# aghasemzadeh/OpenMPL

Hardware: AMD Instinct MI355X
Metric: poses/sec (V=4, J=17, batch=1024 per GPU) fp32 (higher is better)
Workload: dtype f32; 1 GPU; Human3.6M config: V=4 J=17 batch=1024 fp32, CHOSEN flag set, depth 12, DIM 32, heads 8; global_batch=1024, parallelism=single GPU

## Files before the change

### openmpl_amd/csrc/common.hpp

```cpp
#pragma once
#include <stdio.h>
#include <hip/hip_runtime.h>
#include <stdint.h>
#include <stdlib.h>

#include <atomic>
#include <mutex>

#include "../../include/mpl_hip.h"

namespace mpl {

inline const char* lab_getenv(const char* name) {
#ifdef MPL_LAB
    return getenv(name);
#else
    (void)name;
    return nullptr;
#endif
}

typedef _Float16 mpl_f16x8 __attribute__((ext_vector_type(8)));
typedef _Float16 mpl_f16x2 __attribute__((ext_vector_type(2)));
__device__ __forceinline__ void split2_f16(const float (&x)[8], mpl_f16x8& hi, mpl_f16x8& lo) {
    typedef unsigned u4 __attribute__((ext_vector_type(4)));
    u4 h, l;
#pragma unroll
    for (int p = 0; p < 4; ++p) {
        const mpl_f16x2 hp = {(_Float16)x[2 * p], (_Float16)x[2 * p + 1]};
        h[p] = __builtin_bit_cast(unsigned, hp);
        unsigned d;
        asm("v_fma_mixlo_f16 %0, %1, -1.0, %2 op_sel_hi:[1,0,0]\n\t"
            "v_fma_mixhi_f16 %0, %1, -1.0, %3 op_sel:[1,0,0] op_sel_hi:[1,0,0]"
            : "=&v"(d) : "v"(h[p]), "v"(x[2 * p]), "v"(x[2 * p + 1]));
        l[p] = d;
    }
    hi = __builtin_bit_cast(mpl_f16x8, h);
    lo = __builtin_bit_cast(mpl_f16x8, l);
}


typedef float f32x4 __attribute__((ext_vector_type(4)));

constexpr int kWave = 64;

__device__ __forceinline__ f32x4 mfma16(float a, float b, f32x4 c) {
    return __builtin_amdgcn_mfma_f32_16x16x4f32(a, b, c, 0, 0, 0);
}

__device__ __forceinline__ f32x4 mfma16_k16(const float4& a, const float4& b, f32x4 c) {
    c = mfma16(a.x, b.x, c);
    c = mfma16(a.y, b.y, c);
    c = mfma16(a.z, b.z, c);
    c = mfma16(a.w, b.w, c);
    return c;
}

__device__ __forceinline__ float xor16_add(float v) {
    float a = v, b = v;
    asm volatile("s_nop 1\n\tv_permlane16_swap_b32 %0, %1\n\ts_nop 1" : "+v"(a), "+v"(b));
    return a + b;
}
__device__ __forceinline__ float xor32_add(float v) {
    float a = v, b = v;
    asm volatile("s_nop 1\n\tv_permlane32_swap_b32 %0, %1\n\ts_nop 1" : "+v"(a), "+v"(b));
    return a + b;
}

__device__ __forceinline__ float wave_sum(float v) {
#pragma unroll
    for (int o = 32; o > 0; o >>= 1) v += __shfl_xor(v, o, 64);
    return v;
}

__device__ __forceinline__ void dma16(const float* g, unsigned lds_dst) {
    unsigned keep;
    asm volatile(
        "s_mov_b32 %0, m0\n\t"
        "s_mov_b32 m0, %2\n\t"
        "s_nop 0\n\t"
        "global_load_lds_dwordx4 %1, off\n\t"
        "s_mov_b32 m0, %0"
        : "=&s"(keep)
        : "v"(g), "s"(lds_dst)
        : "memory");
}

__device__ __forceinline__ float gelu_erf(float x) { return 0.5f * x * (1.0f + erff(x * 0.70710678118654752440f)); }
__device__ __forceinline__ float gelu_as_scaled(float x, float hs);
__device__ __forceinline__ float gelu_as(float x) { return gelu_as_scaled(x, 0.5f); }
__device__ __forceinline__ float gelu_as_scaled(float x, float hs) {
    const float z = x * 0.70710678118654752440f, az = fabsf(z);
    const float t = __builtin_amdgcn_rcpf(fmaf(0.3275911f, az, 1.0f));
    float pl = fmaf(1.061405429f, t, -1.453152027f);
    pl = fmaf(pl, t, 1.421413741f);
    pl = fmaf(pl, t, -0.284496736f);
    pl = fmaf(pl, t, 0.254829592f);
    const float e = __builtin_amdgcn_exp2f(-1.4426950408889634f * az * az);
    const float h = hs * x, ah = fabsf(h);
    return fmaf(-ah, (pl * t) * e, h + ah);
}


__device__ __forceinline__ float4 ld4(const float* p) { return *reinterpret_cast<const float4*>(p); }
__device__ __forceinline__ void st4(float* p, const float4& v) { *reinterpret_cast<float4*>(p) = v; }

constexpr double FINITE_MAX = 1.79769313486231570e308;
__device__ __forceinline__ bool takes_part(double w) { return w > 0.0 && w <= FINITE_MAX; }

struct ProfScope {
    ProfScope(int kind, hipStream_t s);
    ~ProfScope();
    int slot;
    hipStream_t stream;
};

int device_cu_count(int* cus);

inline int hip_check_launch() {
    hipError_t e = hipGetLastError();
    if (e != hipSuccess) fprintf(stderr, "mpl_hip: kernel launch failed: %s\n", hipGetErrorString(e));
    return e == hipSuccess ? MPL_OK : MPL_E_LAUNCH;
}

template <auto KERNEL>
int kernel_lds_once(int lds, int threads = 0) {
    static std::atomic<bool> done[64];
    int dev = 0;
    if (hipGetDevice(&dev) != hipSuccess || dev < 0 || dev >= 64) return MPL_E_LAUNCH;
    if (done[dev].load(std::memory_order_acquire)) return MPL_OK;
    const void* k = reinterpret_cast<const void*>(KERNEL);
    if (hipFuncSetAttribute(k, hipFuncAttributeMaxDynamicSharedMemorySize, lds) != hipSuccess) return MPL_E_LAUNCH;
    int per_cu = 0;
    if (threads > 0 && (hipOccupancyMaxActiveBlocksPerMultiprocessor(&per_cu, k, threads, lds) != hipSuccess || per_cu < 1))
        return MPL_E_UNSUPPORTED;
    done[dev].store(true, std::memory_order_release);
    return MPL_OK;
}

inline int ln_stat_slices(int K) { return (K % 136 == 0) ? K / 136 : 1; }
int launch_row_stats(const float* x, int M, int K, int ldx, float* stats, hipStream_t s);
int launch_ln_gemm(const float* A, int lda, const float* stats, const float* ln_w, const float* ln_b, float eps,
                   const float* W, const float* bias, const float* R, int ldr, float* C, int ldc, int M, int N, int K,
                   int epi, float* stats_out, hipStream_t s);
bool qkv_attention_fusable(int n_tok, int dim, int heads);
bool ln_gemm_rows_ok(long long M, int K, int lda);
int launch_ln_qkv_attention(const float* x, int M, int D, const float* stats, const float* ln_w, const float* ln_b,
                            float eps, const float* W, const float* bias, int n_tok, int heads, float* att,
                            hipStream_t s);
unsigned* device_error_word(int dev);
int device_error_pending(int dev);
void device_error_clear(int dev);
void set_fault_injection(int phase);
int take_fault_injection();
int refuse_stream_capture(hipStream_t s);
void h2_set_spin_log2(int log2_polls);
int stack_mode();
constexpr int H2_CTR_PER_TILE = 4;
constexpr int H2_XCC_WORDS = 256;
inline int h2_err_index(int n_tiles) { return H2_CTR_PER_TILE * n_tiles + H2_XCC_WORDS; }
int h2_stack_form_code(int M, int D, int n_tok, int np, int cus);
hipEvent_t stack_chain_event(int dev);
std::mutex& stack_chain_mutex(int dev);
bool h2_shape_ok(int N, int K);
size_t h2_operand_bytes(int N, int K, int np = 2);
const float* h2_out_scale(const unsigned short* op, int N, int K);
size_t h2_act_bytes(int M, int K, int rpt, int np = 2);
int h2_rows_per_tile(int n_tok);
bool h2_attention_fusable(int n_tok, int dim, int heads);
void h2_set_debug_buffer(unsigned long long* p);
int launch_pack_h2(const float* W, int N, int K, const float* ln_w, const float* ln_b, const float* bias, const float* in_scale,
                   unsigned short* dst, hipStream_t s);
int launch_h2_entry(const float* X, int M, int K, int ldx, float* stats, unsigned* counters, int n_counters,
                    const unsigned short* const* ops, int n_apps, hipStream_t s);
int launch_h2_pack_rows(const float* X, int M, int K, int ldx, int rpt, unsigned short* dst, float* sc, hipStream_t s);
int launch_h2_gemm(const float* X, const unsigned short* A2, const float* a_inv, const unsigned short* W2, bool ln, const float* stats,
                   float eps, const float* R, int ldr, float* C, int ldc, unsigned short* C2, float* stats_out,
                   int M, int N, int K, int rpt, int epi, hipStream_t s);
int launch_h2_qkv_attention(const float* X, const unsigned short* W2, const float* stats, float eps, int M, int D, int n_tok,
                            int heads, unsigned short* att2, hipStream_t s);
int launch_h2_stack(float* x, int M, int D, int n_tok, int heads, const unsigned short* const* ops, int n_apps,
                    unsigned short* att2, unsigned short* hid2, float* stats, unsigned* counters, float eps, int stop_after,
                    hipStream_t s);
int launch_pack_b1(const float* W, int N, int K, const float* ln_w, const float* ln_b, const float* bias, unsigned short* dst,
                   hipStream_t s);
int launch_b1_entry(const float* X, int M, int K, int ldx, int rpt, unsigned short* x16, float* stats, unsigned* counters,
                    int n_counters, hipStream_t s);
int launch_b1_gemm(const unsigned short* A1, const unsigned short* W1, bool ln, const float* stats, float eps, const float* R, int ldr,
                   float* C, int ldc, unsigned short* C1, float* stats_out, int M, int N, int K, int rpt, int epi, hipStream_t s);
int launch_b1_qkv_attention(const unsigned short* x16, const unsigned short* W1, const float* stats, float eps, int M, int D, int n_tok,
                            int heads, unsigned short* att1, hipStream_t s);
int launch_b1_stack(float* x, unsigned short* x16, int M, int D, int n_tok, int heads, const unsigned short* const* ops, int n_apps,
                    unsigned short* att1, unsigned short* hid1, float* stats, unsigned* counters, float eps, int stop_after,
                    hipStream_t s);
int b1a_ld(int K);
size_t b1a_operand_bytes(int N, int K);
int launch_pack_b1a(const float* W, int N, int K, const float* ln_w, const float* ln_b, const float* bias, unsigned short* dst,
                    hipStream_t s);
int launch_b1a_rows(const float* X, int M, int K, unsigned short* dst, hipStream_t s);
int launch_b1a_gemm(const float* X, int ldx, const unsigned short* A16, int lda, const unsigned short* W16, const float* stats, float eps,
                    const float* R, void* C, int ldc, int M, int N, int K, int epi, hipStream_t s);
bool sm_stack_ok(int M, int D, int n_tok, int H, int n_apps, int n_blocks, int cus);
size_t sm_stack_ws_bytes(int M, int D);
int sm_stack_max_rows();
int launch_sm_stack(float* x, int n_seq, int n_tok, int D, int H, const mpl_block_weights* blocks, const uint8_t* schedule, int n_apps,
                    void* ws, size_t ws_bytes, const unsigned** err_ws, int spin_log2, hipStream_t s);
int launch_token_attention(const float* qkv, int n_seq, int n_tok, int dim, int heads, float* out, hipStream_t s);
bool token_attention_ok(int n_tok, int hd);
bool token_attention_wide_ok(int n_tok, int hd);
int launch_token_attention_wide(const float* qkv, int n_seq, int n_tok, int dim, int heads, float* out, hipStream_t s);
int launch_token_attention_bf16(const float* qkv, int n_seq, int n_tok, int dim, int heads, unsigned short* out16, int ldo, hipStream_t s);
int launch_spt(const mpl_config* cfg, const mpl_weights* w, const mpl_inputs* in, float* xs, int use_packed, hipStream_t s);
int launch_spt_any(const mpl_config* cfg, const mpl_weights* w, const mpl_inputs* in, float* xs, hipStream_t s);
int spt_form(const mpl_config* cfg, int batch, int use_packed, int cus, int* spw);
size_t spt_any_row_bytes(int d);
int spt_any_seq_cap(int J, int d);
size_t spt_pack_bytes();
int launch_spt_pack(const mpl_block_weights* bw_host, unsigned short* dst, int fold_q, hipStream_t s);
int launch_d32_qkv(const float* x, int M, const unsigned short* pack, float* qkv, hipStream_t s);
int launch_d32_mlp(float* x, const float* att, int M, const unsigned short* pack, hipStream_t s);
int launch_fuse_head(const mpl_config* cfg, const mpl_weights* w, const float* x, int batch, float* out, float* y_out,
                     const unsigned* err_ws, hipStream_t s);
int launch_layernorm_rows(const float* x, int M, int K, int ldx, const float* g, const float* b, float eps, float* y,
                          int ldy, hipStream_t s);
int launch_view_norm(const mpl_config* cfg, const mpl_weights* w, const float* x, int batch, float* xn, hipStream_t s);
int launch_linear_act(const float* xa, int Ka, int lda, const float* xb, int Kb, int ldb, int M, const float* W, int ldw,
                      const float* bias, int N, const float* bn_w, const float* bn_b, const float* bn_mean,
                      const float* bn_var, float bn_eps, int relu, float* y, int ldy, hipStream_t s);

int launch_pose_metrics(const float* out, const float* tgt, const float* wgt, int B, int J, const float* scale3,
                        const float* offset3, unsigned skip_mask, float* res, hipStream_t s);

size_t eval_state_bytes(int n_sel, int n_groups);
int launch_eval_reset(void* state, int n_sel, int n_groups, hipStream_t s);
// ... 94 lines not shown
```

### openmpl_amd/csrc/spt_packed.hip

```cpp
#include "spt_pack.hpp"
#include "spt_stage.hpp"

namespace mpl {

constexpr int ATS = 36;
constexpr int HS = 68;
constexpr int KV_F = SJ * SH * SEQ * 4;
constexpr int SPT3_RING_BYTES = (ROWS * XS + 2 * KV_F + ROWS * ATS) * 4;
constexpr int SPT3_LDS_BYTES = 160 * 1024;
constexpr int SPT3_HID_OFF = 3072;
constexpr int SPT3_Q_OFF = 20480;
static_assert(SPT3_HID_OFF + ROWS * HS <= 2 * KV_F + ROWS * ATS, "HID does not fit its alias");
static_assert((SPT3_HID_OFF + ROWS * HS - 2 * KV_F) * 4 <= SPT3_Q_OFF, "HID reaches into the staged qkv weights");
static_assert(SPT3_Q_OFF + 12 * 1024 <= ROWS * ATS * 4, "staged qkv weights do not fit behind HID in ATT");
static_assert(SPT3_RING_BYTES + 8 * 1024 + 2 * SPT3_NPAR * 4 <= SPT3_LDS_BYTES, "spare LDS too small");

typedef float f32x2 __attribute__((ext_vector_type(2)));

__device__ inline float spt_window_scale(float v) {
    if (!(v > 0.f) || !(v < 3.0e38f)) return 1.0f;
    int e;
    (void)frexpf(32768.0f / v, &e);
    e = e - 1 < -100 ? -100 : (e - 1 > 100 ? 100 : e - 1);
    return ldexpf(1.0f, e);
// ... 82 lines not shown
        for (int j = 0; j < 8; ++j) x[j] = src[j] * sw[n];
        sf16x8 hi, lo;
        spt_split2(x, hi, lo);
        frag[(size_t)(u * 2) * 64 + lane] = hi;
        frag[(size_t)(u * 2 + 1) * 64 + lane] = lo;
    }
}

int launch_spt_pack(const mpl_block_weights* bw_host, unsigned short* dst, int fold_q, hipStream_t s) {
    const mpl_block_weights* b = bw_host;
    if (!b || !dst || !b->qkv_w || !b->proj_w || !b->fc1_w || !b->fc2_w || !b->qkv_b || !b->proj_b || !b->fc1_b || !b->fc2_b ||
        !b->ln1_w || !b->ln1_b || !b->ln2_w || !b->ln2_b)
        return MPL_E_INVALID;
    ProfScope prof(MPL_K_PACK, s);
    hipLaunchKernelGGL(spt_pack_kernel, dim3(1), dim3(256), 0, s, b->qkv_w, b->qkv_b, b->ln1_w, b->ln1_b, b->proj_w, b->proj_b, b->fc1_w,
                       b->fc1_b, b->ln2_w, b->ln2_b, b->fc2_w, b->fc2_b, reinterpret_cast<char*>(dst), fold_q);
    return hip_check_launch();
}

size_t spt_pack_bytes() { return SPT_PACK_BYTES; }

template <int N>
struct SptInt { static constexpr int value = N; };

template <int KS, bool LN, bool GELU, int NCT, int AST, int DST, int LO, int HI>
__device__ __forceinline__ void spt_linear_role(const float* A, float* D, const char* wsec, const float* par, int col0, float hs,
                                                int lane) {
    if constexpr (HI > LO) {
        constexpr int M0 = LO / NCT, NM = (HI - 1) / NCT - M0 + 1;
        const int li = lane & 15, kq = lane >> 4;
        sf16x8 w[NCT][KS][2];
        float4 bc[NCT], sc[NCT];
#pragma unroll
        for (int n = 0; n < NCT; ++n) {
            if (HI - LO < NCT && (n - LO % NCT + NCT) % NCT >= HI - LO) continue;
#pragma unroll
            for (int ks = 0; ks < KS; ++ks) spt_load_unit(wsec, n * KS + ks, lane, w[n][ks]);
            bc[n] = ::mpl::ld4(par + col0 + 16 * n + 4 * kq);
            sc[n] = ::mpl::ld4(par + SPT_NCOL + col0 + 16 * n + 4 * kq);
        }
        const float* a0 = A + li * AST + 8 * kq;
        float* d0 = D + li * DST + 4 * kq;
        float4 raw[KS][2], res[NCT];
        auto read_tile = [&](int i) {
            const int m = M0 + i;
#pragma unroll
            for (int ks = 0; ks < KS; ++ks) {
                raw[ks][0] = ::mpl::ld4(a0 + m * 16 * AST + 32 * ks);
                raw[ks][1] = ::mpl::ld4(a0 + m * 16 * AST + 32 * ks + 4);
            }
            if (!GELU) {
#pragma unroll
                for (int n = 0; n < NCT; ++n)
                    if (NCT * m + n >= LO && NCT * m + n < HI) res[n] = ::mpl::ld4(d0 + m * 16 * DST + 16 * n);
            }
        };
        read_tile(0);
#pragma unroll
        for (int i = 0; i < NM; ++i) {
            const int m = M0 + i;
            sf16x8 ah[KS], al[KS];
#pragma unroll
            for (int ks = 0; ks < KS; ++ks) {
                if (LN) {
                    spt_ln_split(raw[ks][0], raw[ks][1], ah[ks], al[ks]);
                } else {
                    const float4 x0 = raw[ks][0], x1 = raw[ks][1];
                    const float y[8] = {x0.x, x0.y, x0.z, x0.w, x1.x, x1.y, x1.z, x1.w};
                    spt_split2(y, ah[ks], al[ks]);
                }
            }
            float4 x[NCT];
#pragma unroll
            for (int n = 0; n < NCT; ++n) x[n] = res[n];
            if (i + 1 < NM) read_tile(i + 1);
            f32x4 c[NCT];
#pragma unroll
            for (int n = 0; n < NCT; ++n) c[n] = f32x4{0.f, 0.f, 0.f, 0.f};
#pragma unroll
            for (int n = 0; n < NCT; ++n) {
                if (NCT * m + n < LO || NCT * m + n >= HI) continue;
#pragma unroll
                for (int ks = 0; ks < KS; ++ks) c[n] = mfma3(w[n][ks], ah[ks], al[ks], c[n]);
            }
#pragma unroll
            for (int n = 0; n < NCT; ++n) {
                if (NCT * m + n < LO || NCT * m + n >= HI) continue;
                float* dd = d0 + m * 16 * DST + 16 * n;
                if (GELU)
                    st4(dd, float4{gelu_as_scaled(fmaf(c[n][0], sc[n].x, bc[n].x), hs), gelu_as_scaled(fmaf(c[n][1], sc[n].y, bc[n].y), hs),
                                   gelu_as_scaled(fmaf(c[n][2], sc[n].z, bc[n].z), hs), gelu_as_scaled(fmaf(c[n][3], sc[n].w, bc[n].w), hs)});
                else
                    st4(dd, float4{x[n].x + fmaf(c[n][0], sc[n].x, bc[n].x), x[n].y + fmaf(c[n][1], sc[n].y, bc[n].y),
                                   x[n].z + fmaf(c[n][2], sc[n].z, bc[n].z), x[n].w + fmaf(c[n][3], sc[n].w, bc[n].w)});
            }
        }
    }
}
#define SPT_ROLE(W, MTS, KS, LN, GELU, NCT, AST, DST, ...) \
    spt_linear_role<KS, LN, GELU, NCT, AST, DST, ((MTS) * (NCT) * (W)) / NWAVE, ((MTS) * (NCT) * ((W) + 1)) / NWAVE>(__VA_ARGS__)
#define SPT_BY_WAVE(wv, ...)                          \
    switch (wv) {                                     \
        case 0: SPT_ROLE(0, __VA_ARGS__); break;      \
        case 1: SPT_ROLE(1, __VA_ARGS__); break;      \
        case 2: SPT_ROLE(2, __VA_ARGS__); break;      \
        case 3: SPT_ROLE(3, __VA_ARGS__); break;      \
        case 4: SPT_ROLE(4, __VA_ARGS__); break;      \
        case 5: SPT_ROLE(5, __VA_ARGS__); break;      \
        case 6: SPT_ROLE(6, __VA_ARGS__); break;      \
        default: SPT_ROLE(7, __VA_ARGS__); break;     \
    }


template <int SS>
__global__ __launch_bounds__(NTHR, 1) void spt3_kernel(const SptParams p) {
    constexpr int RLIVE = SJ * SS;
    constexpr int MTS = (RLIVE + 15) / 16;
    constexpr int NT = (MTS + 3) / 4;
    extern __shared__ __attribute__((aligned(16))) float smem[];
    float* X = smem;
    float* Kb = smem + ROWS * XS;
    float* Vb = Kb + KV_F;
    float* ATT = Vb + KV_F;
    float* HID = Kb + SPT3_HID_OFF;
    char* S_W = reinterpret_cast<char*>(ATT + ROWS * ATS);
    float* S_PAR = reinterpret_cast<float*>(S_W + 8 * 1024);
    char* R_F1 = reinterpret_cast<char*>(Kb);
    char* R_Q = reinterpret_cast<char*>(ATT) + SPT3_Q_OFF;

    const int tid = threadIdx.x, lane = tid & 63;
    const int wave = __builtin_amdgcn_readfirstlane(tid >> 6);
    const int li = lane & 15, kq = lane >> 4;
    auto phase_sync = [&]() {
        asm volatile("s_waitcnt vmcnt(0)" ::: "memory");
        __syncthreads();
    };
    const int hg = wave & 1, part = wave >> 1;
    const int view = blockIdx.x % p.V;
    const int b0 = (blockIdx.x / p.V) * SS;
    const int sl = li % SS;
    const mpl_spt_set set = p.sets[(p.flags & MPL_F_MULTI_SPT) ? view : 0];
    const float* pose = p.poses[view];
    const float* ray = p.rays[view];
    const float* cen = p.centers[view];

    auto stage_w = [&](char* dst, const unsigned short* pack, int byte_off, int n_pieces) {
        const unsigned l0 = (unsigned)(uintptr_t)(__attribute__((address_space(3))) char*)dst;
        for (int i = wave; i < n_pieces; i += NWAVE)
            ::mpl::dma16(reinterpret_cast<const float*>(reinterpret_cast<const char*>(pack) + byte_off + i * 1024) + lane * 4,
                         l0 + (unsigned)(i * 1024));
    };
    auto load_par = [&](const mpl_block_weights& b) -> float4 {
        if (tid >= SPT3_NPAR / 4) return float4{0.f, 0.f, 0.f, 0.f};
        return ld4(G(reinterpret_cast<const float*>(reinterpret_cast<const char*>(b.qkv_w3) + SPT_PACK_VEC)) + 4 * tid);
    };
    auto store_par = [&](int app_of, const float4& v) {
        if (tid < SPT3_NPAR / 4) st4(S_PAR + (app_of & 1) * SPT3_NPAR + 4 * tid, v);
    };
    mpl_block_weights bw;
    if (p.n_apps > 0) {
        bw = set.blocks[p.sched[0] & 0x7f];
        stage_w(R_Q, bw.qkv_w3, SPT_PACK_QKV, 12);
    }
    const float4 par0 = p.n_apps > 0 ? load_par(bw) : float4{0.f, 0.f, 0.f, 0.f};
    spt_embed<true, SS>(p, set, X, tid, b0, pose, ray, cen, SS, MTS * 16);
    store_par(0, par0);
    phase_sync();

    auto load_w = [&](const char* region, int unit, sf16x8 (&w)[2]) { spt_load_unit(region, unit, lane, w); };
    auto ln_frag = [&](int m, sf16x8& ah, sf16x8& al) {
        const float* xr = X + (m * 16 + li) * XS + 8 * kq;
        spt_ln_split(::mpl::ld4(xr), ::mpl::ld4(xr + 4), ah, al);
    };
    for (int app = 0; app < p.n_apps; ++app) {
        const bool weighted = (p.sched[app] & 0x80) != 0;
        bw = set.blocks[p.sched[app] & 0x7f];
        const unsigned short* pack = bw.qkv_w3;
        const float* par = S_PAR + (app & 1) * SPT3_NPAR;
        stage_w(S_W, pack, SPT_PACK_PROJ, 4);
        {
            sf16x8 wq[3][2];
            float4 bq[3], sq[3];
#pragma unroll
            for (int c = 0; c < 3; ++c) {
                load_w(R_Q, 2 * c + hg, wq[c]);
                bq[c] = ::mpl::ld4(par + SPT_C_QKV + 32 * c + 16 * hg + 4 * kq);
                sq[c] = ::mpl::ld4(par + SPT_NCOL + SPT_C_QKV + 32 * c + 16 * hg + 4 * kq);
            }
            float4 q[NT];
#pragma unroll
            for (int t = 0; t < NT; ++t) {
                q[t] = float4{0.f, 0.f, 0.f, 0.f};
                if (part + 4 * t < MTS && !(p.abl & 8)) {
                    const int m = part + 4 * t;
                    const int j = (16 * m + li) / SS;
                    const bool live = 16 * m + li < RLIVE;
                    sf16x8 ah, al;
                    ln_frag(m, ah, al);
                    const f32x4 z = {0.f, 0.f, 0.f, 0.f};
                    const f32x4 cq = mfma3(wq[0], ah, al, z), ck = mfma3(wq[1], ah, al, z), cv = mfma3(wq[2], ah, al, z);
                    q[t] = float4{fmaf(cq[0], sq[0].x, bq[0].x), fmaf(cq[1], sq[0].y, bq[0].y), fmaf(cq[2], sq[0].z, bq[0].z),
                                  fmaf(cq[3], sq[0].w, bq[0].w)};
                    const int h = 4 * hg + kq;
                    const float kx = fmaf(ck[0], sq[1].x, bq[1].x), ky = fmaf(ck[1], sq[1].y, bq[1].y);
                    const float kz = fmaf(ck[2], sq[1].z, bq[1].z), kw = fmaf(ck[3], sq[1].w, bq[1].w);
                    if (live && j < SJ - 1) {
                        float* kp = Kb + ((((j >> 1) * 2) * SH + h) * SS + sl) * 4 + (j & 1);
                        kp[0] = kx;
                        kp[2] = ky;
                        kp[SH * SS * 4] = kz;
                        kp[SH * SS * 4 + 2] = kw;
                    } else if (live) {
                        st4(Kb + (SJ - 1) * SH * SS * 4 + (h * SS + sl) * 4, float4{kx, ky, kz, kw});
                    }
                    if (live)
                        st4(Vb + ((j * SH + h) * SS + sl) * 4, float4{fmaf(cv[0], sq[2].x, bq[2].x), fmaf(cv[1], sq[2].y, bq[2].y),
                                                                       fmaf(cv[2], sq[2].z, bq[2].z), fmaf(cv[3], sq[2].w, bq[2].w)});
                }
            }
            phase_sync();
            auto attention = [&](auto live_tiles) {
                constexpr int NL = decltype(live_tiles)::value;
                const int h = 4 * hg + kq;
                float sc[NL][SJ];
#pragma unroll
                for (int jp = 0; jp < SJ / 2; ++jp) {
                    const float4 k01 = ::mpl::ld4(Kb + (((jp * 2) * SH + h) * SS + sl) * 4);
                    const float4 k23 = ::mpl::ld4(Kb + (((jp * 2 + 1) * SH + h) * SS + sl) * 4);
                    const f32x2 kx = {k01.x, k01.y}, ky = {k01.z, k01.w}, kz = {k23.x, k23.y}, kw = {k23.z, k23.w};
#pragma unroll
                    for (int t = 0; t < NL; ++t) {
                        const f32x2 qx = {q[t].x, q[t].x}, qy = {q[t].y, q[t].y}, qz = {q[t].z, q[t].z}, qw = {q[t].w, q[t].w};
                        f32x2 s2 = qx * kx;
                        s2 = __builtin_elementwise_fma(qy, ky, s2);
                        s2 = __builtin_elementwise_fma(qz, kz, s2);
                        s2 = __builtin_elementwise_fma(qw, kw, s2);
                        sc[t][2 * jp] = s2[0];
                        sc[t][2 * jp + 1] = s2[1];
                    }
                }
                {
                    const float4 k = ::mpl::ld4(Kb + (SJ - 1) * SH * SS * 4 + (h * SS + sl) * 4);
#pragma unroll
                    for (int t = 0; t < NL; ++t)
                        sc[t][SJ - 1] = fmaf(q[t].w, k.w, fmaf(q[t].z, k.z, fmaf(q[t].y, k.y, q[t].x * k.x)));
                }
                const float s_att = par[2 * SPT_NCOL];
                const float* conf0 = nullptr;
                if (weighted) {
                    int l16 = li;
                    asm volatile("" : "+v"(l16));
                    conf0 = pose + ((size_t)(b0 + l16 % SS) * SJ + (16 * part + l16) / SS) * 3 + 2;
                }
                float inv[NL];
#pragma unroll
                for (int t = 0; t < NL; ++t) {
                    float mx = sc[t][0];
#pragma unroll
                    for (int j = 1; j < SJ; ++j) mx = fmaxf(mx, sc[t][j]);
                    float l = 0.f;
#pragma unroll
                    for (int j = 0; j < SJ; ++j) {
                        sc[t][j] = __builtin_amdgcn_exp2f(sc[t][j] - mx);
                        l += sc[t][j];
                    }
                    inv[t] = __builtin_amdgcn_rcpf(l) * s_att;
                    if (weighted) {
                        const int b = b0 + sl, r = 16 * (part + 4 * t) + li;
                        inv[t] *= (b < p.B && r < RLIVE) ? conf0[3 * (64 / SS) * t] : 0.f;
                    }
                }
                float4 o[NL];
#pragma unroll
                for (int t = 0; t < NL; ++t) o[t] = float4{0.f, 0.f, 0.f, 0.f};
#pragma unroll
                for (int j = 0; j < SJ; ++j) {
                    const float4 v = ::mpl::ld4(Vb + ((j * SH + h) * SS + sl) * 4);
#pragma unroll
                    for (int t = 0; t < NL; ++t) {
                        const float pj = sc[t][j];
                        o[t].x = fmaf(pj, v.x, o[t].x);
                        o[t].y = fmaf(pj, v.y, o[t].y);
                        o[t].z = fmaf(pj, v.z, o[t].z);
                        o[t].w = fmaf(pj, v.w, o[t].w);
                    }
                }
#pragma unroll
                for (int t = 0; t < NL; ++t) {
                    o[t] = float4{o[t].x * inv[t], o[t].y * inv[t], o[t].z * inv[t], o[t].w * inv[t]};
                    if (weighted) {
                        const float big = fmaxf(fmaxf(fabsf(o[t].x), fabsf(o[t].y)), fmaxf(fabsf(o[t].z), fabsf(o[t].w)));
                        if (!(big <= 65000.f)) {
                            const float qn = __builtin_nanf("");
                            o[t] = float4{qn, qn, qn, qn};
                            if (big < __builtin_inff() && p.err_host)
                                __hip_atomic_fetch_or(p.err_host, 2u, __ATOMIC_RELAXED, __HIP_MEMORY_SCOPE_SYSTEM);
                        }
                    }
                }
#pragma unroll
                for (int t = 0; t < NL; ++t) st4(ATT + ((part + 4 * t) * 16 + li) * ATS + 4 * h, o[t]);
            };
            if (!(p.abl & 1)) {
                if (part + 4 * (NT - 1) < MTS) attention(SptInt<NT>{});
                else if (NT > 1) attention(SptInt<(NT > 1 ? NT - 1 : 1)>{});
            }
        }
        phase_sync();
        stage_w(R_F1, pack, SPT_PACK_FC1, 8);
        if (!(p.abl & 32)) SPT_BY_WAVE(wave, MTS, 1, false, false, 2, ATS, XS, ATT, X, S_W, par, SPT_C_PROJ, 0.f, lane);
        phase_sync();
        stage_w(S_W, pack, SPT_PACK_FC2, 8);
        if (!(p.abl & 64))
            SPT_BY_WAVE(wave, MTS, 1, true, true, 4, XS, HS, X, HID, R_F1, par, SPT_C_FC1, par[2 * SPT_NCOL + 1], lane);
        phase_sync();
        {
            float4 parn = float4{0.f, 0.f, 0.f, 0.f};
            if (app + 1 < p.n_apps) {
                const mpl_block_weights bn = set.blocks[p.sched[app + 1] & 0x7f];
                stage_w(R_Q, bn.qkv_w3, SPT_PACK_QKV, 12);
                parn = load_par(bn);
            }
            if (!(p.abl & 128)) SPT_BY_WAVE(wave, MTS, 2, false, false, 2, HS, XS, HID, X, S_W, par, SPT_C_FC2, 0.f, lane);
            if (app + 1 < p.n_apps) store_par(app + 1, parn);
        }
        phase_sync();
    }
    spt_epilogue<true, SS>(p, X, tid, view, b0, pose, ray, cen, SS, MTS * 16);
}

template <int SS>
static int launch_spt3(const SptParams& p, int grid, hipStream_t s) {
    if (int rc = kernel_lds_once<spt3_kernel<SS>>(SPT3_LDS_BYTES)) return rc;
    hipLaunchKernelGGL(spt3_kernel<SS>, dim3(grid), dim3(NTHR), SPT3_LDS_BYTES, s, p);
    return hip_check_launch();
}

int launch_spt_packed(const SptParams& p, int ss, int grid, hipStream_t s) {
    switch (ss) {
        case 1: return launch_spt3<1>(p, grid, s);
        case 2: return launch_spt3<2>(p, grid, s);
        case 4: return launch_spt3<4>(p, grid, s);
        case 8: return launch_spt3<8>(p, grid, s);
        case 16: return launch_spt3<16>(p, grid, s);
        default: return MPL_E_INVALID;
    }
}

}
```

### openmpl_amd/csrc/spt_stage.hpp

```cpp
#pragma once
#include "common.hpp"

namespace mpl {

constexpr int SJ = 17;
constexpr int SD = 32;
constexpr int SH = 8;
constexpr int SEQ = 16;
constexpr int ROWS = SEQ * SJ;
constexpr int XS = 36;
constexpr int NTHR = 512;
constexpr int NWAVE = NTHR / 64;
constexpr int SPT_SMALL_SPW = 8;

struct SptParams {
    const float* poses[MPL_MAX_VIEWS];
    const float* rays[MPL_MAX_VIEWS];
    const float* centers[MPL_MAX_VIEWS];
    const mpl_spt_set* sets;
    const float *snorm_w, *snorm_b;
    const float *pos3d_embed, *pos3d_view, *pos3d_lin_w, *pos3d_lin_b;
    const float *ray_w, *ray_b, *cfpt_w, *cfpt_b;
    float* xs;
    int B, V, in_ch, n_apps;
    unsigned flags;
    int c3;
    int spw;
    int abl;
    unsigned* err_host;
    unsigned char sched[MPL_MAX_APPS];
};

int launch_spt_native(const SptParams& p, int form, int grid, hipStream_t s);
int launch_spt_packed(const SptParams& p, int ss, int grid, hipStream_t s);

typedef const __attribute__((address_space(1))) float* gfp;
__device__ __forceinline__ gfp G(const float* p) { return (gfp)p; }
__device__ __forceinline__ float4 ld4(gfp p) {
    typedef float v4 __attribute__((ext_vector_type(4)));
    const v4 t = *reinterpret_cast<const __attribute__((address_space(1))) v4*>(p);
    return make_float4(t.x, t.y, t.z, t.w);
}

template <bool TM, int SS = SEQ>
__device__ __forceinline__ void row_to_sj(int r, int& sq, int& j) {
    if (TM) { j = r / SS; sq = r % SS; }
    else { sq = r / SJ; j = r - sq * SJ; }
}

template <bool TM, int SS = SEQ>
__device__ __forceinline__ void spt_embed(const SptParams& p, const mpl_spt_set& set, float* X, int tid, int b0,
                                          const float* pose, const float* ray, const float* cen, int nseq = SEQ, int nrows = ROWS) {
    for (int idx = tid; idx < nrows * SD; idx += NTHR) {
        const int r = idx >> 5, c = idx & 31;
        int sq, j;
        row_to_sj<TM, SS>(r, sq, j);
        const int b = b0 + sq;
        float x = 0.f;
        if (b < p.B && sq < nseq && j < SJ) {
            const float* in = pose + ((size_t)b * SJ + j) * 3;
            const float* we = set.embed_w + c * p.in_ch;
            x = set.embed_b[c] + we[0] * in[0] + we[1] * in[1];
            if (p.in_ch == 3) x += we[2] * in[2];
            if (p.flags & MPL_F_CONF_ADD) x += set.conf_w[c] * in[2] + set.conf_b[c];
            if (p.flags & MPL_F_CONF_MULT) x *= set.conf_w[c] * in[2] + set.conf_b[c];
            x += set.pos_embed[j * SD + c];
            if (p.flags & MPL_F_POS3D_SPATIAL) {
                if (p.flags & MPL_F_POS3D_LEARN) {
                    x += p.pos3d_embed[j * p.c3 + c];
                } else {
                    const float* rr = ray + ((size_t)b * SJ + j) * 3;
                    const float* cc = cen + (size_t)b * 3;
                    const float vx = rr[0] - cc[0], vy = rr[1] - cc[1], vz = rr[2] - cc[2];
                    const float nrm = fmaxf(sqrtf(vx * vx + vy * vy + vz * vz), 1e-12f);
                    const float* wl = p.pos3d_lin_w + c * 3;
                    x += p.pos3d_lin_b[c] + wl[0] * (vx / nrm) + wl[1] * (vy / nrm) + wl[2] * (vz / nrm);
                }
            }
        }
        X[r * XS + c] = x;
    }
}

template <bool TM, int SS = SEQ>
__device__ __forceinline__ void spt_epilogue(const SptParams& p, const float* X, int tid, int view, int b0, const float* pose,
                                             const float* ray, const float* cen, int nseq = SEQ, int nrows = ROWS) {
    const bool to_rays = (p.flags & MPL_F_POS3D_TO_RAYS) && (p.flags & MPL_F_RAYS_TOKEN);
    const bool ray_tok = !(p.flags & MPL_F_POS3D_TO_RAYS) && (p.flags & MPL_F_RAYS_TOKEN);
    const int cw = to_rays ? 2 * SD : SD;
    const int Df = SJ * SD * ((p.flags & MPL_F_RAYS_TOKEN) ? 2 : 1);
    for (int r = tid; r < nrows; r += NTHR) {
        int sq, j;
        row_to_sj<TM, SS>(r, sq, j);
        const int b = b0 + sq;
        if (b >= p.B || sq >= nseq || j >= SJ) continue;
        const float* xr = X + r * XS;
        float v[SD];
        float s = 0.f;
#pragma unroll
        for (int c = 0; c < SD; c += 4) {
            const float4 t = ld4(xr + c);
            v[c] = t.x; v[c + 1] = t.y; v[c + 2] = t.z; v[c + 3] = t.w;
            s += (t.x + t.y) + (t.z + t.w);
        }
        const float mean = s * (1.0f / 32.0f);
        float ss = 0.f;
#pragma unroll
        for (int c = 0; c < SD; ++c) {
            v[c] -= mean;
            ss = fmaf(v[c], v[c], ss);
        }
        const float rstd = 1.0f / sqrtf(ss * (1.0f / 32.0f) + 1e-6f);
        const float conf = pose[((size_t)b * SJ + j) * 3 + 2];
        float dx = 0.f, dy = 0.f, dz = 0.f, nx = 0.f, ny = 0.f, nz = 0.f;
        const bool need_dir = (p.flags & MPL_F_RAYS_TOKEN) ||
                              (!(p.flags & MPL_F_POS3D_SPATIAL) && !(p.flags & MPL_F_POS3D_LEARN));
        if (need_dir) {
            const float* rr = ray + ((size_t)b * SJ + j) * 3;
            const float* cc = cen + (size_t)b * 3;
            dx = rr[0] - cc[0]; dy = rr[1] - cc[1]; dz = rr[2] - cc[2];
            const float nrm = fmaxf(sqrtf(dx * dx + dy * dy + dz * dz), 1e-12f);
            nx = dx / nrm; ny = dy / nrm; nz = dz / nrm;
        }
        auto pos3d = [=](int c) -> float {
            if (p.flags & MPL_F_POS3D_SPATIAL) return p.pos3d_view[j * p.c3 + c];
            if (p.flags & MPL_F_POS3D_LEARN) return p.pos3d_embed[j * p.c3 + c];
            const float* wl = p.pos3d_lin_w + c * 3;
            return p.pos3d_lin_b[c] + wl[0] * nx + wl[1] * ny + wl[2] * nz;
        };
        auto ray_emb = [=](int c) -> float {
            const float* wr = p.ray_w + c * 3;
            return p.ray_b[c] + wr[0] * dx + wr[1] * dy + wr[2] * dz;
        };
        float* orow = p.xs + ((size_t)b * p.V + view) * Df;
        float* o1 = orow + j * cw;
#pragma unroll
        for (int c = 0; c < SD; c += 4) {
            float t[4];
#pragma unroll
            for (int q = 0; q < 4; ++q) {
                float y = v[c + q] * rstd * p.snorm_w[c + q] + p.snorm_b[c + q];
                if (p.flags & MPL_F_CONF_IN_FPT) y += p.cfpt_w[c + q] * conf + p.cfpt_b[c + q];
                t[q] = y + pos3d(c + q);
            }
            st4(o1 + c, float4{t[0], t[1], t[2], t[3]});
        }
        if (to_rays) {
#pragma unroll
            for (int c = 0; c < SD; c += 4) {
                float t[4];
#pragma unroll
                for (int q = 0; q < 4; ++q) t[q] = ray_emb(c + q) + pos3d(SD + c + q);
                st4(o1 + SD + c, float4{t[0], t[1], t[2], t[3]});
            }
        } else if (ray_tok) {
            float* o2 = orow + (SJ + j) * SD;
#pragma unroll
            for (int c = 0; c < SD; c += 4) st4(o2 + c, float4{ray_emb(c), ray_emb(c + 1), ray_emb(c + 2), ray_emb(c + 3)});
        }
    }
}

}
```

Before: 848,300 poses/s.

## Prefetch embed inputs into registers and stage epilogue operands into LDS via DMA

The embed step now loads its global operands into registers (Spt3Embed::load) before the first weight staging and writes them into X afterwards, so those global reads overlap the qkv weight DMA. During the last block application, the epilogue's per-row operands (norm params, conf, rays, centers, pos3d tables) are DMA'd into the free K-buffer region of LDS with a new global_load_lds_dword helper. The epilogue is also rewritten so 8 threads share each row, each handling 4 columns, and it reads those operands from LDS instead of scattered global loads. This adds register pressure, extra LDS aliasing constraints and some fp-contract changes that could shift numerics slightly.

```diff
diff --git a/openmpl_amd/csrc/common.hpp b/openmpl_amd/csrc/common.hpp
--- a/openmpl_amd/csrc/common.hpp
+++ b/openmpl_amd/csrc/common.hpp
@@ -80,6 +80,19 @@
         "s_mov_b32 m0, %2\n\t"
         "s_nop 0\n\t"
         "global_load_lds_dwordx4 %1, off\n\t"
+        "s_mov_b32 m0, %0"
+        : "=&s"(keep)
+        : "v"(g), "s"(lds_dst)
+        : "memory");
+}
+
+__device__ __forceinline__ void dma4(const float* g, unsigned lds_dst) {
+    unsigned keep;
+    asm volatile(
+        "s_mov_b32 %0, m0\n\t"
+        "s_mov_b32 m0, %2\n\t"
+        "s_nop 0\n\t"
+        "global_load_lds_dword %1, off\n\t"
         "s_mov_b32 m0, %0"
         : "=&s"(keep)
         : "v"(g), "s"(lds_dst)
diff --git a/openmpl_amd/csrc/spt_packed.hip b/openmpl_amd/csrc/spt_packed.hip
--- a/openmpl_amd/csrc/spt_packed.hip
+++ b/openmpl_amd/csrc/spt_packed.hip
@@ -258,18 +258,32 @@
     };
     auto load_par = [&](const mpl_block_weights& b) -> float4 {
         if (tid >= SPT3_NPAR / 4) return float4{0.f, 0.f, 0.f, 0.f};
-        return ld4(G(reinterpret_cast<const float*>(reinterpret_cast<const char*>(b.qkv_w3) + SPT_PACK_VEC)) + 4 * tid);
+        int t = tid;
+        asm volatile("" : "+v"(t));
+        return ld4(G(reinterpret_cast<const float*>(reinterpret_cast<const char*>(b.qkv_w3) + SPT_PACK_VEC)) + 4 * t);
     };
     auto store_par = [&](int app_of, const float4& v) {
         if (tid < SPT3_NPAR / 4) st4(S_PAR + (app_of & 1) * SPT3_NPAR + 4 * tid, v);
     };
+    float* ENDS = Kb;
+    typedef const __attribute__((address_space(4))) SptParams* kparg;
+    auto stage_ends = [&]() {
+        kparg kp = (kparg)__builtin_amdgcn_kernarg_segment_ptr();
+        asm volatile("" : "+s"(kp));
+        const SptParams& q = *(const SptParams*)kp;
+        spt3_stage_ends<SS>(q, ENDS, wave, lane, (int)(blockIdx.x % q.V), (int)(blockIdx.x / q.V) * SS);
+    };
+    Spt3Embed<SS> emb;
+    emb.load(p, set, tid, b0, pose, ray, cen);
     mpl_block_weights bw;
     if (p.n_apps > 0) {
         bw = set.blocks[p.sched[0] & 0x7f];
         stage_w(R_Q, bw.qkv_w3, SPT_PACK_QKV, 12);
+    } else {
+        stage_ends();
     }
     const float4 par0 = p.n_apps > 0 ? load_par(bw) : float4{0.f, 0.f, 0.f, 0.f};
-    spt_embed<true, SS>(p, set, X, tid, b0, pose, ray, cen, SS, MTS * 16);
+    emb.store(p, X, tid, b0);
     store_par(0, par0);
     phase_sync();
 
@@ -294,13 +308,15 @@
                 sq[c] = ::mpl::ld4(par + SPT_NCOL + SPT_C_QKV + 32 * c + 16 * hg + 4 * kq);
             }
             float4 q[NT];
+            int lq = li;
+            asm volatile("" : "+v"(lq));
 #pragma unroll
             for (int t = 0; t < NT; ++t) {
                 q[t] = float4{0.f, 0.f, 0.f, 0.f};
                 if (part + 4 * t < MTS && !(p.abl & 8)) {
                     const int m = part + 4 * t;
-                    const int j = (16 * m + li) / SS;
-                    const bool live = 16 * m + li < RLIVE;
+                    const int j = (16 * m + lq) / SS;
+                    const bool live = 16 * m + lq < RLIVE;
                     sf16x8 ah, al;
                     ln_frag(m, ah, al);
                     const f32x4 z = {0.f, 0.f, 0.f, 0.f};
@@ -353,9 +369,9 @@
                 }
                 const float s_att = par[2 * SPT_NCOL];
                 const float* conf0 = nullptr;
+                int l16 = li;
+                asm volatile("" : "+v"(l16));
                 if (weighted) {
-                    int l16 = li;
-                    asm volatile("" : "+v"(l16));
                     conf0 = pose + ((size_t)(b0 + l16 % SS) * SJ + (16 * part + l16) / SS) * 3 + 2;
                 }
                 float inv[NL];
@@ -372,8 +388,8 @@
                     }
                     inv[t] = __builtin_amdgcn_rcpf(l) * s_att;
                     if (weighted) {
-                        const int b = b0 + sl, r = 16 * (part + 4 * t) + li;
-                        inv[t] *= (b < p.B && r < RLIVE) ? conf0[3 * (64 / SS) * t] : 0.f;
+                        const int b = b0 + l16 % SS, r = 16 * (part + 4 * t) + l16;
+                        inv[t] *= (b < p.B && (RLIVE % 16 == 0 || r < RLIVE)) ? conf0[3 * (64 / SS) * t] : 0.f;
                     }
                 }
                 float4 o[NL];
@@ -426,13 +442,20 @@
                 const mpl_block_weights bn = set.blocks[p.sched[app + 1] & 0x7f];
                 stage_w(R_Q, bn.qkv_w3, SPT_PACK_QKV, 12);
                 parn = load_par(bn);
+            } else {
+                stage_ends();
             }
             if (!(p.abl & 128)) SPT_BY_WAVE(wave, MTS, 2, false, false, 2, HS, XS, HID, X, S_W, par, SPT_C_FC2, 0.f, lane);
             if (app + 1 < p.n_apps) store_par(app + 1, parn);
         }
         phase_sync();
     }
-    spt_epilogue<true, SS>(p, X, tid, view, b0, pose, ray, cen, SS, MTS * 16);
+    {
+        kparg kp = (kparg)__builtin_amdgcn_kernarg_segment_ptr();
+        asm volatile("" : "+s"(kp));
+        const SptParams& q = *(const SptParams*)kp;
+        spt3_epilogue<SS>(q, X, ENDS, tid, (int)(blockIdx.x % q.V), (int)(blockIdx.x / q.V) * SS);
+    }
 }
 
 template <int SS>
diff --git a/openmpl_amd/csrc/spt_stage.hpp b/openmpl_amd/csrc/spt_stage.hpp
--- a/openmpl_amd/csrc/spt_stage.hpp
+++ b/openmpl_amd/csrc/spt_stage.hpp
@@ -161,4 +161,287 @@
     }
 }
 
-}
+
+constexpr int SE_SNORM = 0;
+constexpr int SE_CFPT = 64;
+constexpr int SE_RAYW = 128;
+constexpr int SE_RAYB = 224;
+constexpr int SE_LINW = 256;
+constexpr int SE_LINB = 448;
+constexpr int SE_POS3D = 512;
+constexpr int SE_CONF = 1600;
+constexpr int SE_RAY = 1920;
+constexpr int SE_CEN = 2752;
+constexpr int SE_FLOATS = 2816;
+static_assert(SE_FLOATS * 4 <= 12 * 1024, "the staged epilogue operands reach into HID");
+
+template <int SS>
+__device__ __forceinline__ void spt3_stage_ends(const SptParams& p, float* E, int wave, int lane, int view, int b0) {
+    constexpr int RLIVE = SJ * SS;
+    asm volatile("" : "+v"(lane), "+s"(wave));
+    const float* pose = p.poses[view];
+    const float* ray = p.rays[view];
+    const float* cen = p.centers[view];
+    const unsigned f = p.flags;
+    const bool rays_tok = (f & MPL_F_RAYS_TOKEN) != 0;
+    const bool to_rays = (f & MPL_F_POS3D_TO_RAYS) && rays_tok;
+    const bool tab = (f & (MPL_F_POS3D_SPATIAL | MPL_F_POS3D_LEARN)) != 0;
+    const bool need_dir = rays_tok || !tab;
+    const int cw = to_rays ? 2 * SD : SD;
+    const int blast = p.B - 1;
+    const unsigned e0 = (unsigned)(uintptr_t)(__attribute__((address_space(3))) float*)E;
+    for (int pc = wave; pc < SE_FLOATS / 64; pc += NWAVE) {
+        const float* src = pose;
+        bool on = false;
+        if (pc < 2) {
+            const float* w = pc ? p.cfpt_w : p.snorm_w;
+            const float* o = pc ? p.cfpt_b : p.snorm_b;
+            asm volatile("" : "+s"(w), "+s"(o));
+            on = pc == 0 || (f & MPL_F_CONF_IN_FPT) != 0;
+            src = (lane < 32 ? w : o) + (lane & 31);
+        } else if (pc < 4) {
+            const int k = (pc - 2) * 64 + lane;
+            on = rays_tok;
+            src = k < 3 * SD ? p.ray_w + k : p.ray_b + (k - 3 * SD);
+        } else if (pc < 8) {
+            const int k = (pc - 4) * 64 + lane;
+            on = !tab;
+            src = k < 192 ? p.pos3d_lin_w + (k < 3 * cw ? k : 0) : p.pos3d_lin_b + (k - 192 < cw ? k - 192 : 0);
+        } else if (pc < 25) {
+            on = tab;
+            src = ((f & MPL_F_POS3D_SPATIAL) ? p.pos3d_view : p.pos3d_embed) + (pc - 8) * p.c3 + (lane < cw ? lane : 0);
+        } else if (pc < 30) {
+            int r = (pc - 25) * 64 + lane;
+            r = r < RLIVE ? r : RLIVE - 1;
+            int b = b0 + r % SS;
+            b = b < blast ? b : blast;
+            on = true;
+            src = pose + ((size_t)b * SJ + r / SS) * 3 + 2;
+        } else if (pc < 43) {
+            const int k = (pc - 30) * 64 + lane;
+            int r = k / 3;
+            const int comp = k - 3 * r;
+            r = r < RLIVE ? r : RLIVE - 1;
+            int b = b0 + r % SS;
+            b = b < blast ? b : blast;
+            on = need_dir;
+            src = ray + ((size_t)b * SJ + r / SS) * 3 + comp;
+        } else {
+            const int k = lane < 3 * SS ? lane : 3 * SS - 1;
+            int b = b0 + k / 3;
+            b = b < blast ? b : blast;
+            on = need_dir;
+            src = cen + (size_t)b * 3 + k % 3;
+        }
+        if (on) dma4(src, e0 + (unsigned)(pc * 256));
+    }
+}
+
+template <int SS>
+struct Spt3Embed {
+    static constexpr int RLIVE = SJ * SS;
+    static constexpr int MTS = (RLIVE + 15) / 16;
+    float w0, w1, w2, eb, cfw, cfb, wl0, wl1, wl2, lb, c0, c1, c2;
+    float in0[MTS], in1[MTS], in2[MTS], pe[MTS], e0[MTS], e1[MTS], e2[MTS];
+
+    __device__ __forceinline__ void load(const SptParams& p, const mpl_spt_set& set, int tid, int b0, const float* pose,
+                                         const float* ray, const float* cen) {
+        const int c = tid & 31, r0 = tid >> 5;
+        const int b = b0 + r0 % SS;
+        const int bc = b < p.B ? b : p.B - 1;
+        const unsigned f = p.flags;
+        const bool conf = (f & (MPL_F_CONF_ADD | MPL_F_CONF_MULT)) != 0;
+        const bool learn = (f & MPL_F_POS3D_SPATIAL) && (f & MPL_F_POS3D_LEARN);
+        const bool lin = (f & MPL_F_POS3D_SPATIAL) && !(f & MPL_F_POS3D_LEARN);
+        const gfp we = G(set.embed_w) + c * p.in_ch;
+        w0 = we[0];
+        w1 = we[1];
+        w2 = 0.f;
+        if (p.in_ch == 3) w2 = we[2];
+        eb = G(set.embed_b)[c];
+        cfw = cfb = 0.f;
+        if (conf) {
+            cfw = G(set.conf_w)[c];
+            cfb = G(set.conf_b)[c];
+        }
+        wl0 = wl1 = wl2 = lb = c0 = c1 = c2 = 0.f;
+        if (lin) {
+            const gfp wl = G(p.pos3d_lin_w) + c * 3;
+            wl0 = wl[0];
+            wl1 = wl[1];
+            wl2 = wl[2];
+            lb = G(p.pos3d_lin_b)[c];
+            const gfp cc = G(cen) + (size_t)bc * 3;
+            c0 = cc[0];
+            c1 = cc[1];
+            c2 = cc[2];
+        }
+#pragma unroll
+        for (int i = 0; i < MTS; ++i) {
+            const int j = (r0 + 16 * i) / SS, jc = j < SJ ? j : SJ - 1;
+            const gfp in = G(pose) + ((size_t)bc * SJ + jc) * 3;
+            in0[i] = in[0];
+            in1[i] = in[1];
+            in2[i] = in[2];
+            pe[i] = G(set.pos_embed)[jc * SD + c];
+            e0[i] = e1[i] = e2[i] = 0.f;
+        }
+        if (learn) {
+#pragma unroll
+            for (int i = 0; i < MTS; ++i) {
+                const int j = (r0 + 16 * i) / SS, jc = j < SJ ? j : SJ - 1;
+                e0[i] = G(p.pos3d_embed)[jc * p.c3 + c];
+            }
+        }
+        if (lin) {
+#pragma unroll
+            for (int i = 0; i < MTS; ++i) {
+                const int j = (r0 + 16 * i) / SS, jc = j < SJ ? j : SJ - 1;
+                const gfp rr = G(ray) + ((size_t)bc * SJ + jc) * 3;
+                e0[i] = rr[0];
+                e1[i] = rr[1];
+                e2[i] = rr[2];
+            }
+        }
+    }
+
+    __device__ __forceinline__ void store(const SptParams& p, float* X, int tid, int b0) const {
+#pragma clang fp contract(off)
+        const int c = tid & 31, r0 = tid >> 5;
+        const bool bl = b0 + r0 % SS < p.B;
+        const unsigned f = p.flags;
+        const bool in3 = p.in_ch == 3, cadd = (f & MPL_F_CONF_ADD) != 0, cmul = (f & MPL_F_CONF_MULT) != 0;
+        const bool learn = (f & MPL_F_POS3D_SPATIAL) && (f & MPL_F_POS3D_LEARN);
+        const bool lin = (f & MPL_F_POS3D_SPATIAL) && !(f & MPL_F_POS3D_LEARN);
+#pragma unroll
+        for (int i = 0; i < MTS; ++i) {
+            const int r = r0 + 16 * i;
+            float x = (eb + w0 * in0[i]) + w1 * in1[i];
+            if (in3) x = fmaf(w2, in2[i], x);
+            if (cadd) x = x + fmaf(cfw, in2[i], cfb);
+            if (cmul) x = x * fmaf(cfw, in2[i], cfb);
+            x = x + pe[i];
+            if (learn) x = x + e0[i];
+            if (lin) {
+                const float vx = e0[i] - c0, vy = e1[i] - c1, vz = e2[i] - c2;
+                const float nrm = fmaxf(sqrtf(fmaf(vx, vx, vy * vy) + vz * vz), 1e-12f);
+                x = x + ((fmaf(wl0, vx / nrm, lb) + wl1 * (vy / nrm)) + wl2 * (vz / nrm));
+            }
+            X[r * XS + c] = (bl && r < RLIVE) ? x : 0.f;
+        }
+    }
+};
+
+template <int SS>
+__device__ __forceinline__ void spt3_epilogue(const SptParams& p, const float* X, const float* E, int tid, int view, int b0) {
+#pragma clang fp contract(off)
+    constexpr int RLIVE = SJ * SS;
+    asm volatile("" : "+v"(tid));
+    const unsigned f = p.flags;
+    const bool rays_tok = (f & MPL_F_RAYS_TOKEN) != 0;
+    const bool to_rays = (f & MPL_F_POS3D_TO_RAYS) && rays_tok;
+    const bool ray_tok = !(f & MPL_F_POS3D_TO_RAYS) && rays_tok;
+    const bool tab = (f & (MPL_F_POS3D_SPATIAL | MPL_F_POS3D_LEARN)) != 0;
+    const bool need_dir = rays_tok || !tab;
+    const bool cfpt = (f & MPL_F_CONF_IN_FPT) != 0;
+    const int cw = to_rays ? 2 * SD : SD;
+    const int Df = SJ * SD * (rays_tok ? 2 : 1);
+    const int q0 = 4 * (tid & 7);
+    const float4 z4 = float4{0.f, 0.f, 0.f, 0.f};
+    const float4 sw = ld4(E + SE_SNORM + q0), sb = ld4(E + SE_SNORM + SD + q0);
+    float4 fw = z4, fb = z4, rb = z4, lb = z4, lb2 = z4;
+    float wr[4][3] = {}, wl[4][3] = {}, wl2[4][3] = {};
+    if (cfpt) {
+        fw = ld4(E + SE_CFPT + q0);
+        fb = ld4(E + SE_CFPT + SD + q0);
+    }
+    if (rays_tok) {
+        rb = ld4(E + SE_RAYB + q0);
+        const float4 a = ld4(E + SE_RAYW + 3 * q0), b = ld4(E + SE_RAYW + 3 * q0 + 4), c = ld4(E + SE_RAYW + 3 * q0 + 8);
+        wr[0][0] = a.x; wr[0][1] = a.y; wr[0][2] = a.z; wr[1][0] = a.w; wr[1][1] = b.x; wr[1][2] = b.y;
+        wr[2][0] = b.z; wr[2][1] = b.w; wr[2][2] = c.x; wr[3][0] = c.y; wr[3][1] = c.z; wr[3][2] = c.w;
+    }
+    if (!tab) {
+        lb = ld4(E + SE_LINB + q0);
+        const float4 a = ld4(E + SE_LINW + 3 * q0), b = ld4(E + SE_LINW + 3 * q0 + 4), c = ld4(E + SE_LINW + 3 * q0 + 8);
+        wl[0][0] = a.x; wl[0][1] = a.y; wl[0][2] = a.z; wl[1][0] = a.w; wl[1][1] = b.x; wl[1][2] = b.y;
+        wl[2][0] = b.z; wl[2][1] = b.w; wl[2][2] = c.x; wl[3][0] = c.y; wl[3][1] = c.z; wl[3][2] = c.w;
+        if (to_rays) {
+            lb2 = ld4(E + SE_LINB + SD + q0);
+            const float4 d = ld4(E + SE_LINW + 3 * (SD + q0)), e = ld4(E + SE_LINW + 3 * (SD + q0) + 4),
+                         g = ld4(E + SE_LINW + 3 * (SD + q0) + 8);
+            wl2[0][0] = d.x; wl2[0][1] = d.y; wl2[0][2] = d.z; wl2[1][0] = d.w; wl2[1][1] = e.x; wl2[1][2] = e.y;
+            wl2[2][0] = e.z; wl2[2][1] = e.w; wl2[2][2] = g.x; wl2[3][0] = g.y; wl2[3][1] = g.z; wl2[3][2] = g.w;
+        }
+    }
+    for (int r = tid >> 3; r < RLIVE; r += NTHR / 8) {
+        const int j = r / SS, sq = r % SS, b = b0 + sq;
+        if (b >= p.B) continue;
+        const float* xr = X + r * XS;
+        float v[SD];
+        float s = 0.f;
+#pragma unroll
+        for (int c = 0; c < SD; c += 4) {
+            const float4 t = ld4(xr + c);
+            v[c] = t.x; v[c + 1] = t.y; v[c + 2] = t.z; v[c + 3] = t.w;
+            s += (t.x + t.y) + (t.z + t.w);
+        }
+        float ss = 0.f;
+#pragma unroll
+        for (int c = 0; c < SD; ++c) {
+            v[c] = fmaf(s, -1.0f / 32.0f, v[c]);
+            ss = fmaf(v[c], v[c], ss);
+        }
+        const float rstd = 1.0f / sqrtf(fmaf(ss, 1.0f / 32.0f, 1e-6f));
+        const float4 mq = ld4(xr + q0);
+        const float m[4] = {fmaf(s, -1.0f / 32.0f, mq.x), fmaf(s, -1.0f / 32.0f, mq.y), fmaf(s, -1.0f / 32.0f, mq.z),
+                            fmaf(s, -1.0f / 32.0f, mq.w)};
+        const float conf = E[SE_CONF + r];
+        float dx = 0.f, dy = 0.f, dz = 0.f, nx = 0.f, ny = 0.f, nz = 0.f;
+        if (need_dir) {
+            const float* rr = E + SE_RAY + 3 * r;
+            const float* cc = E + SE_CEN + 3 * sq;
+            dx = rr[0] - cc[0]; dy = rr[1] - cc[1]; dz = rr[2] - cc[2];
+            const float nrm = fmaxf(sqrtf(fmaf(dx, dx, dy * dy) + dz * dz), 1e-12f);
+            nx = dx / nrm; ny = dy / nrm; nz = dz / nrm;
+        }
+        float4 p1 = z4, p2 = z4;
+        if (tab) {
+            p1 = ld4(E + SE_POS3D + j * 64 + q0);
+            if (to_rays) p2 = ld4(E + SE_POS3D + j * 64 + SD + q0);
+        } else {
+            const float4 lbv[2] = {lb, lb2};
+            float o[2][4];
+#pragma unroll
+            for (int h = 0; h < 2; ++h) {
+                const float bq[4] = {lbv[h].x, lbv[h].y, lbv[h].z, lbv[h].w};
+#pragma unroll
+                for (int q = 0; q < 4; ++q) {
+                    const float* w = h ? wl2[q] : wl[q];
+                    o[h][q] = (fmaf(w[0], nx, bq[q]) + w[1] * ny) + w[2] * nz;
+                }
+            }
+            p1 = float4{o[0][0], o[0][1], o[0][2], o[0][3]};
+            if (to_rays) p2 = float4{o[1][0], o[1][1], o[1][2], o[1][3]};
+        }
+        const float swq[4] = {sw.x, sw.y, sw.z, sw.w}, sbq[4] = {sb.x, sb.y, sb.z, sb.w};
+        const float fwq[4] = {fw.x, fw.y, fw.z, fw.w}, fbq[4] = {fb.x, fb.y, fb.z, fb.w};
+        const float p1q[4] = {p1.x, p1.y, p1.z, p1.w}, p2q[4] = {p2.x, p2.y, p2.z, p2.w};
+        const float rbq[4] = {rb.x, rb.y, rb.z, rb.w};
+        float t[4], re[4];
+#pragma unroll
+        for (int q = 0; q < 4; ++q) {
+            float y = fmaf(m[q] * rstd, swq[q], sbq[q]);
+            if (cfpt) y = y + fmaf(fwq[q], conf, fbq[q]);
+            t[q] = y + p1q[q];
+            re[q] = fmaf(wr[q][2], dz, fmaf(wr[q][1], dy, fmaf(wr[q][0], dx, rbq[q])));
+        }
+        float* orow = p.xs + ((size_t)b * p.V + view) * Df;
+        float* o1 = orow + j * cw;
+        st4(o1 + q0, float4{t[0], t[1], t[2], t[3]});
+        if (to_rays) st4(o1 + SD + q0, float4{re[0] + p2q[0], re[1] + p2q[1], re[2] + p2q[2], re[3] + p2q[3]});
+        else if (ray_tok) st4(orow + (SJ + j) * SD + q0, float4{re[0], re[1], re[2], re[3]});
+    }
+}
+
+}
```

Result: no change. 850,800 poses/s (median of 6 runs) (+0.3%).
